# JingyunLiang/HCFlow

Measured on AMD Instinct MI355X. Metric: HR images/sec (inverse sample) DIV2K x4 160px LR, higher is better.
Workload: dtype f32 via f16x3 split (hi/lo f16 products, f32 accumulate); 1 GPU; SR_DF2K_4X inverse sampling (netG reverse=True), batch 16/GPU, LR 160x160 -> HR 640x640, tau=0.8, eps on device, output all-gather over RCCL for N>1; global_batch=16, lr_size=160, parallelism=dp1, streams_per_gpu=2

## Files before the change

hcflow_amd/csrc/hcf_conv_wino.h:

```cpp
#pragma once
#include <hip/hip_runtime.h>
#include <stdint.h>
#include <string.h>
#include <math.h>
#include <type_traits>
#include <vector>

namespace hcf {
namespace wino {

constexpr int TW = 32, TH = 8, HWP = TW + 2, HHP = TH + 2;
constexpr int A_REAL_PIECES = HHP * HWP * 4;
constexpr int A_BYTES = 22 * 1024;
constexpr int W_BYTES = 16 * 2 * 2 * 32 * 16;
constexpr int STAGE = A_BYTES + W_BYTES;
constexpr int X_BYTES = 10240;
constexpr int S0_OFF = 0, X_OFF = STAGE, S1_OFF = STAGE + X_BYTES, TAB_OFF = S1_OFF + STAGE;
constexpr int LDS_BYTES = TAB_OFF + 512;
constexpr float UNSPLIT = 1.f / 2048.f;

struct Src { const float* p; int cs, c0, n; };
struct Args {
  Src src[3];
  int nsrc;
// ... 128 lines not shown
  const int R = px >> 2, sl = (px & 3) * 4 + part;
  return R * 256 + ((sl ^ ((R & 7) << 1)) << 4);
}


namespace v2 {
constexpr int TH2 = 16, HH2 = TH2 + 2;
constexpr int A2_REAL = HH2 * HWP * 4;
constexpr int A2_BYTES = 39 * 1024;
constexpr int STAGE2 = A2_BYTES + W_BYTES;
constexpr int TAB2_OFF = 2 * STAGE2;
constexpr int LDS2_BYTES = TAB2_OFF + 512;
constexpr int FB2_OFF = LDS2_BYTES;
constexpr int LDS2S_BYTES = FB2_OFF + 512 * 16 + 64;
constexpr int ROWB = HWP * 64;
__host__ __device__ constexpr int a2_off(int row, int x, int part) {
  return row * ROWB + (x >> 2) * 256 + (((((x & 3) * 4 + part)) ^ ((x >> 2) & 7)) << 4);
}
}

typedef _Float16 f16x2 __attribute__((ext_vector_type(2)));
typedef uint32_t u32x4 __attribute__((ext_vector_type(4)));
__device__ __forceinline__ void split8(const float (&v)[8], u32x4& h, u32x4& l) {
#pragma unroll
  for (int i = 0; i < 4; ++i) {
    const f16x2 hh = {(_Float16)v[2 * i], (_Float16)v[2 * i + 1]};
    h[i] = __builtin_bit_cast(uint32_t, hh);
    uint32_t lo;
    asm("v_fma_mixlo_f16 %0, %1, -1.0, %2 op_sel_hi:[1,0,0]" : "=v"(lo) : "v"(h[i]), "v"(v[2 * i]));
    asm("v_fma_mixhi_f16 %0, %1, -1.0, %2 op_sel:[1,0,0] op_sel_hi:[1,0,0]" : "+v"(lo) : "v"(h[i]), "v"(v[2 * i + 1]));
// ... 28 lines not shown
}

typedef uint32_t u32x2 __attribute__((ext_vector_type(2)));
__device__ __forceinline__ void split4(const f32x4& v, u32x2& h, u32x2& l) {
#pragma unroll
  for (int i = 0; i < 2; ++i) {
    const f16x2 hh = {(_Float16)v[2 * i], (_Float16)v[2 * i + 1]};
    h[i] = __builtin_bit_cast(uint32_t, hh);
    uint32_t lo;
    asm("v_fma_mixlo_f16 %0, %1, -1.0, %2 op_sel_hi:[1,0,0]" : "=v"(lo) : "v"(h[i]), "v"(v[2 * i]));
    asm("v_fma_mixhi_f16 %0, %1, -1.0, %2 op_sel:[1,0,0] op_sel_hi:[1,0,0]" : "+v"(lo) : "v"(h[i]), "v"(v[2 * i + 1]));
    l[i] = lo;
  }
}

template <int RES, bool SC = false>
__global__ __launch_bounds__(512, 1) void conv_wino2_kernel(const Args a, const int nunits) {
  using namespace v2;
  extern __shared__ __attribute__((aligned(16))) char lds[];
  const int tid = threadIdx.x, lane = tid & 63, half = lane >> 5, li = lane & 31;
  const int wave = __builtin_amdgcn_readfirstlane(tid >> 6);
  const int xp = wave & 1, tg = wave >> 1;
  const int H = a.H, W = a.W, ntn = a.ntile_n, nchunk = a.nchunk;
  const int tiles_x = (W + TW - 1) / TW, tiles_y = (H + TH2 - 1) / TH2;

  const bool w7 = (wave == 7);
  const int padpix = a.B * H * W;
  int upix[5];
#pragma unroll
  for (int j = 0; j < 5; ++j) upix[j] = padpix;
  uint32_t partpk = 0;
#pragma unroll
  for (int j = 0; j < 5; ++j) {
// ... 52 lines not shown
  {                                                                                                \
    const int p16_ = (int)((pp_ >> (2 * (J))) & 0x30u);                                            \
    const int vo_ = (int)__umul24((unsigned)upix[J], (unsigned)csb_) + p16_;                       \
    W2_DMA(rsa_, vo_, so_, DST);                                                                   \
  }
#define W2_ISSUE(J0, J1, STG)                                                                      \
  {                                                                                                \
    char* const sb_ = lds + (STG) * STAGE2 + wave * 1024;                                          \
    _Pragma("unroll") for (int j_ = (J0); j_ < (J1); ++j_) {                                       \
      if (j_ < 4) W2_A_SLOT(j_ < 5 ? j_ : 0, sb_ + j_ * 8192)                                      \
      else if (j_ == 4) { if (!w7) W2_A_SLOT(4, sb_ + 4 * 8192) else W2_DMA(rsw, wvo, ws_, sb_ + 4 * 8192); } \
      else if (j_ < 8) W2_DMA(rsw, wvo, ws_ + (8 * j_ + wave - 39) * 1024, sb_ + j_ * 8192);       \
      else if (!w7) W2_DMA(rsw, wvo, ws_ + (8 * 8 + wave - 39) * 1024, sb_ + 8 * 8192);            \
    }                                                                                              \
  }

  const int trow = li >> 4, tcol = li & 15;
  int poff[4];
#pragma unroll
  for (int j = 0; j < 4; ++j) poff[j] = a2_off(4 * tg + 2 * trow, 2 * tcol + j, 2 * half);
  const int rowP = xp ? ROWB : 0, rowS = xp ? 3 * ROWB : 2 * ROWB;
  const float sg = __builtin_bit_cast(float, __builtin_amdgcn_readfirstlane(__builtin_bit_cast(int, xp ? -1.f : 1.f)));
  const int fw = A2_BYTES + half * 512 + li * 16 + xp * (8 * 4 * 512);

  float in_s = 1.f, out_s = 1.f;
  int in_max_bits = 0;
  if (SC) input_scales(a.in_max, in_s, out_s, in_max_bits);
  constexpr bool FBK = SC && RES == 0;
  const bool fb = FBK && a.fb_y != nullptr;
  if (tid < 64) {
    const float sc_ = (tid < 32 * ntn) ? a.scale[tid] : 1.f, bi_ = (tid < 32 * ntn) ? a.bias[tid] : 0.f;
    reinterpret_cast<float*>(lds + TAB2_OFF)[tid] = bi_ * sc_;
    reinterpret_cast<float*>(lds + TAB2_OFF)[64 + tid] = sc_ * UNSPLIT * out_s;
  }
  if (FBK) {
    if (fb) {
      *reinterpret_cast<f32x4*>(lds + FB2_OFF + tid * 16) = f32x4{0.f, 0.f, 0.f, 0.f};
      if (tid == 0) *reinterpret_cast<int*>(lds + FB2_OFF + 512 * 16) = 0;
    }
  }
  int u = blockIdx.x;
  if (u >= nunits) return;
#if defined(WINO_PROF)
  unsigned long long pw[8] = {0, 0, 0, 0, 0, 0, 0, 0};
  const unsigned long long pw_t0 = __builtin_readcyclecounter();
#endif
  W2_SETUP_UNIT(u)
  W2_CHUNK_SCALARS()
  W2_ISSUE(0, 9, 0)
  ++uc;
  int g = 0;
  const float slope = a.act == 1 ? 0.f : a.act == 2 ? 0.2f : 1.f;

  while (true) {
    f32x16 acc[8];
#pragma unroll
    for (int p = 0; p < 8; ++p)
#pragma unroll
      for (int r = 0; r < 16; ++r) acc[p][r] = 0.f;
    const int eb = ub, ey0 = uy0, ex0 = ux0, ent = unt;
    const int un = u + gridDim.x;

    for (int c = 0; c < nchunk; ++c, ++g) {
      const int stg = g & 1;
#if defined(WINO_PROF)
      const unsigned long long q0 = __builtin_readcyclecounter();
#endif
      asm volatile("s_waitcnt vmcnt(0)" ::: "memory");
#if defined(WINO_PROF)
      const unsigned long long q1 = __builtin_readcyclecounter();
#endif
      __builtin_amdgcn_s_barrier();
#if defined(WINO_PROF)
      const unsigned long long q2 = __builtin_readcyclecounter();
      pw[0] += q1 - q0; pw[1] += q2 - q1;
#endif
      if (c + 1 == nchunk) {
        if (un < nunits) W2_SETUP_UNIT(un)
        else {
          uc = 0; unt = 0;
#pragma unroll
          for (int j = 0; j < 5; ++j) upix[j] = padpix;
        }
      }
      W2_CHUNK_SCALARS()
      const char* const sb = lds + stg * STAGE2;
      const int so = stg ^ 1;
#define W2_LOAD_ROW(D, OFF)                                                                        \
  _Pragma("unroll") for (int j = 0; j < 4; ++j) {                                                  \
    const f32x4 x0_ = *reinterpret_cast<const f32x4*>(sb + poff[j] + (OFF));                       \
    const f32x4 x1_ = *reinterpret_cast<const f32x4*>(sb + (poff[j] ^ 16) + (OFF));                \
    _Pragma("unroll") for (int k = 0; k < 4; ++k) { D[j][k] = x0_[k]; D[j][4 + k] = x1_[k]; }      \
  }
#define W2_V(NU, T, K) (((NU) == 0) ? T[0][K] - T[2][K] : ((NU) == 1) ? T[1][K] + T[2][K] : ((NU) == 2) ? T[1][K] - T[2][K] : T[1][K] - T[3][K])
#define W2_MFMA(P, WW, VX) acc[P] = __builtin_amdgcn_mfma_f32_32x32x16_f16(WW, __builtin_bit_cast(f16x8, VX), acc[P], 0, 0, 0);
#define W2_XI(I, T)                                                                                \
  _Pragma("unroll") for (int nu = 0; nu < 4; ++nu) {                                               \
    float v_[8];                                                                                   \
    _Pragma("unroll") for (int k = 0; k < 8; ++k) v_[k] = W2_V(nu, T, k);                          \
    u32x4 vh_, vl_;                                                                                \
    if (SC) split8s(v_, in_s, vh_, vl_); else split8(v_, vh_, vl_);                                \
    const f16x8 w1_ = *reinterpret_cast<const f16x8*>(sb + fw + (((I) * 4 + nu) * 4) * 512);       \
    const f16x8 w2_ = *reinterpret_cast<const f16x8*>(sb + fw + (((I) * 4 + nu) * 4 + 2) * 512);   \
    W2_MFMA((I) * 4 + nu, w1_, vh_)                                                                \
    W2_MFMA((I) * 4 + nu, w2_, vh_)                                                                \
    W2_MFMA((I) * 4 + nu, w1_, vl_)                                                                \
  }
      float t_[4][8];
      {
        float ra[4][8], rc[4][8];
        W2_LOAD_ROW(ra, rowP)
        W2_LOAD_ROW(rc, 2 * ROWB)
        W2_ISSUE(0, 3, so)
#pragma unroll
        for (int j = 0; j < 4; ++j)
#pragma unroll
          for (int k = 0; k < 8; ++k) t_[j][k] = ra[j][k] - rc[j][k];
      }
      W2_XI(0, t_)
      W2_ISSUE(3, 6, so)
      {
        float ra[4][8], rc[4][8];
        W2_LOAD_ROW(ra, ROWB)
        W2_LOAD_ROW(rc, rowS)
#pragma unroll
        for (int j = 0; j < 4; ++j)
#pragma unroll
          for (int k = 0; k < 8; ++k) t_[j][k] = fmaf(sg, rc[j][k], ra[j][k]);
      }
      W2_ISSUE(6, 9, so)
      ++uc;
      W2_XI(1, t_)
#if defined(WINO_PROF)
      pw[6] += __builtin_readcyclecounter() - q2;
#endif
#undef W2_XI
#undef W2_MFMA
#undef W2_V
#undef W2_LOAD_ROW
    }

#if defined(WINO_PROF)
    const unsigned long long qe0 = __builtin_readcyclecounter();
#endif
    float chk = 0.f;
    f32x4 fbs = {0.f, 0.f, 0.f, 0.f};
    float fbm = 0.f;
    {
      char* const xbuf = lds + ((g - 1) & 1) * STAGE2 + tg * 16384;
      const int p8 = lane >> 3, qd = (lane >> 1) & 3, hd = lane & 1;
      const int wpos = (half * 32 + ((li + 4 * half) & 31)) * 16;
      const int wpos1 = (half * 32 + ((li + 4 * half + 8) & 31)) * 16;
      const int cb = ent * 32 + 8 * qd + 4 * hd;
      const f32x4 bs = *reinterpret_cast<const f32x4*>(lds + TAB2_OFF + cb * 4);
      const f32x4 ms = *reinterpret_cast<const f32x4*>(lds + TAB2_OFF + 256 + cb * 4);
      const bool second = (RES == 0) && a.out2 != nullptr && cb >= a.out2_split;
      const float slope_l = second ? (a.act2 == 1 ? 0.f : a.act2 == 2 ? 0.2f : 1.f) : slope;
      __builtin_amdgcn_s_barrier();
#pragma unroll
      for (int oa = 0; oa < 2; ++oa) {
        f32x4 rv1[2][2], rv2[2][2];
        size_t pixs[2][2];
        bool oks[2][2];
        int rpos[2];
#pragma unroll
        for (int sgrp = 0; sgrp < 2; ++sgrp) {
          const int patch = 16 * xp + 8 * sgrp + p8, prow = patch >> 4, pcol = patch & 15;
          rpos[sgrp] = (hd * 32 + ((patch + 4 * hd + 8 * (qd & 1)) & 31)) * 16 + qd * 1024;
#pragma unroll
          for (int ob = 0; ob < 2; ++ob) {
            const int yy = ey0 + 4 * tg + 2 * prow + oa, xx = ex0 + 2 * pcol + ob;
            oks[sgrp][ob] = yy < H && xx < W;
            pixs[sgrp][ob] = (size_t)((size_t)eb * H + (yy < H ? yy : H - 1)) * W + (xx < W ? xx : W - 1);
            if (RES == 1 || RES == 2) rv1[sgrp][ob] = *reinterpret_cast<const f32x4*>(a.res1 + pixs[sgrp][ob] * a.res1_cs + a.res1_c0 + cb);
            if (RES == 2) rv2[sgrp][ob] = *reinterpret_cast<const f32x4*>(a.res2 + pixs[sgrp][ob] * a.res2_cs + a.res2_c0 + cb);
            if (RES == 3) rv1[sgrp][ob] = *reinterpret_cast<const f32x4*>(a.pre + pixs[sgrp][ob] * a.pre_cs + a.pre_c0 + cb);
            if (FBK) { if (fb) rv1[sgrp][ob] = *reinterpret_cast<const f32x4*>(a.fb_y + pixs[sgrp][ob] * a.fb_y_cs + a.fb_y_c0 + cb); }
          }
        }
        if (oa == 1) __builtin_amdgcn_s_barrier();
#pragma unroll
        for (int q = 0; q < 4; ++q) {
          f32x4 P[2];
#pragma unroll
          for (int e = 0; e < 4; ++e) {
            const int r = 4 * q + e;
            float R[2][2];
#pragma unroll
            for (int i = 0; i < 2; ++i) {
              R[i][0] = acc[i * 4 + 0][r] + acc[i * 4 + 1][r] + acc[i * 4 + 2][r];
              R[i][1] = acc[i * 4 + 1][r] - acc[i * 4 + 2][r] - acc[i * 4 + 3][r];
            }
#pragma unroll
            for (int bb = 0; bb < 2; ++bb)
              P[bb][e] = (oa == 0) ? (xp ? R[0][bb] : R[0][bb] + R[1][bb]) : (xp ? -R[0][bb] - R[1][bb] : R[1][bb]);
          }
          char* const wbq = xbuf + ((xp * 2) * 4 + q) * 1024 + ((q & 1) ? wpos1 : wpos);
          *reinterpret_cast<f32x4*>(wbq) = P[0];
          *reinterpret_cast<f32x4*>(wbq + 4096) = P[1];
        }
        __builtin_amdgcn_s_barrier();
#pragma unroll
        for (int sgrp = 0; sgrp < 2; ++sgrp)
#pragma unroll
          for (int ob = 0; ob < 2; ++ob) {
            const f32x4 y0 = *reinterpret_cast<const f32x4*>(xbuf + ((0 * 2 + ob) * 4) * 1024 + rpos[sgrp]);
            const f32x4 y1 = *reinterpret_cast<const f32x4*>(xbuf + ((1 * 2 + ob) * 4) * 1024 + rpos[sgrp]);
            f32x4 v;
#pragma unroll
            for (int e = 0; e < 4; ++e) {
              const float yv = y0[e] + y1[e];
              chk = fmaf(yv, 0.f, chk);
              float z = fmaf(yv, ms[e], bs[e]);
              if (RES == 3) z = fmaf(rv1[sgrp][ob][e], ms[e] * 2048.f, z);
              v[e] = fmaxf(z, slope_l * z);
              if (RES == 1 || RES == 2) v[e] = fmaf(v[e], a.rs1, rv1[sgrp][ob][e]);
// ... 48 lines not shown
        }
      }
      if (tid == 0) {
        const int m = *reinterpret_cast<const int*>(lds + FB2_OFF + 512 * 16), m2 = max(m, in_max_bits);
        if (a.fb_max && m) atomicMax(reinterpret_cast<int*>(a.fb_max), m);
        if (a.fb_max2 && m2) atomicMax(reinterpret_cast<int*>(a.fb_max2), m2);
      }
    }
  }
#if defined(WINO_PROF)
  if (a.dbg && lane == 0 && (blockIdx.x & 31) == 17) {
    atomicAdd(a.dbg + 0, pw[0]); atomicAdd(a.dbg + 1, pw[1]); atomicAdd(a.dbg + 2, __builtin_readcyclecounter() - pw_t0);
    atomicAdd(a.dbg + 3, pw[3]); atomicAdd(a.dbg + 4, 1ull); atomicAdd(a.dbg + 5, pw[5]); atomicAdd(a.dbg + 6, pw[6]);
  }
#endif
#undef W2_SETUP_UNIT
#undef W2_DMA
#undef W2_A_SLOT
#undef W2_ISSUE
#undef W2_CHUNK_SCALARS
}

namespace v4 {
constexpr int TH4 = 8, HH4 = TH4 + 2;
constexpr int A4_BYTES = 22 * 1024;
constexpr int W4L_BYTES = 48 * 1024;
constexpr int W4_OFF0 = 2 * A4_BYTES;
constexpr int X4_SPARE = 19 * 1024;
constexpr int W4_OFF1 = W4_OFF0 + W4L_BYTES + X4_SPARE;
constexpr int TAB4_OFF = W4_OFF1 + W4L_BYTES;
constexpr int LDS4_BYTES = TAB4_OFF + 1024;
constexpr int NPIECE4 = 22 + 48;
}

// ... 346 lines not shown
    a.clk[3] = __builtin_amdgcn_s_memrealtime();
  }
  f16x8 w11[4];
  W4_SETUP_UNIT(u)
  W4_CHUNK_SCALARS()
  W4_ISSUE_A(0)
  W4_ISSUE_W(2, 9, 0)
#pragma unroll
  for (int nu = 0; nu < 4; ++nu) W4_LOAD_W11(nu)
  ++uc;
  int g = 0;
  const float slope = a.act == 1 ? 0.f : a.act == 2 ? 0.2f : 1.f;
  const float slope2 = a.act2 == 1 ? 0.f : a.act2 == 2 ? 0.2f : 1.f;
  const float slope_f = a.f_act == 1 ? 0.f : a.f_act == 2 ? 0.2f : 1.f;

  while (true) {
    f32x16 acc[4][2];
#pragma unroll
    for (int p = 0; p < 4; ++p)
#pragma unroll
      for (int n = 0; n < 2; ++n)
#pragma unroll
        for (int r = 0; r < 16; ++r) acc[p][n][r] = 0.f;
    const int eb = ub, ey0 = uy0, ex0 = ux0;
    const int un = u + gridDim.x;

    for (int c = 0; c < nchunk; ++c, ++g) {
      const int stg = g & 1;
#if defined(WINO_PROF)
      const unsigned long long q0 = __builtin_readcyclecounter();
#endif
      if (c > 0 || g == 0 || a.top_wait) asm volatile("s_waitcnt vmcnt(0)" ::: "memory");
#if defined(WINO_PROF)
      const unsigned long long q1 = __builtin_readcyclecounter();
#endif
      __builtin_amdgcn_s_barrier();
#if defined(WINO_PROF)
      const unsigned long long q2 = __builtin_readcyclecounter();
      pw[0] += q1 - q0; pw[1] += q2 - q1;
      if (c == 0 && g > 0) { pw[21] += q1 - q0; pw[22] += q2 - q1; pw[23] += 1; }
#endif
#pragma unroll
      for (int nu = 0; nu < 4; ++nu) asm volatile("" : "+v"(w11[nu]));
      if (c + 1 == nchunk) {
        if (un < nunits) W4_SETUP_UNIT(un)
        else {
          uc = 0;
#pragma unroll
          for (int j = 0; j < 3; ++j) upix[j] = padpix;
        }
      }
      W4_CHUNK_SCALARS()
      W4_ISSUE_A((g + 1) & 1)
      float t_[4][8];
      {
        const char* const ib = lds + (g & 1) * A4_BYTES;
        float ra[4][8], rb[4][8];
#pragma unroll
        for (int j = 0; j < 4; ++j) {
          const f32x4 x0_ = *reinterpret_cast<const f32x4*>(ib + poff[j] + offA);
          const f32x4 x1_ = *reinterpret_cast<const f32x4*>(ib + (poff[j] ^ 16) + offA);
          const f32x4 y0_ = *reinterpret_cast<const f32x4*>(ib + poff[j] + offB);
          const f32x4 y1_ = *reinterpret_cast<const f32x4*>(ib + (poff[j] ^ 16) + offB);
#pragma unroll
          for (int k = 0; k < 4; ++k) { ra[j][k] = x0_[k]; ra[j][4 + k] = x1_[k]; rb[j][k] = y0_[k]; rb[j][4 + k] = y1_[k]; }
        }
#pragma unroll
        for (int j = 0; j < 4; ++j)
#pragma unroll
          for (int k = 0; k < 8; ++k) t_[j][k] = fmaf(sg, rb[j][k], ra[j][k]);
      }
#if defined(WINO_PROF)
      const unsigned long long q3 = __builtin_readcyclecounter();
      pw[5] += q3 - q2;
#endif
      const char* const wb = lds + (stg ? W4_OFF1 : W4_OFF0) + fw;
#define W4_V(NU, K) (((NU) == 0) ? t_[0][K] - t_[2][K] : ((NU) == 1) ? t_[1][K] + t_[2][K] : ((NU) == 2) ? t_[1][K] - t_[2][K] : t_[1][K] - t_[3][K])
#define W4_MFMA(P, N, WW, VX) acc[P][N] = __builtin_amdgcn_mfma_f32_32x32x16_f16(WW, __builtin_bit_cast(f16x8, VX), acc[P][N], 0, 0, 0);
#pragma unroll
      for (int nu = 0; nu < 4; ++nu) {
        float v_[8];
#pragma unroll
        for (int k = 0; k < 8; ++k) v_[k] = W4_V(nu, k);
        u32x4 vh_, vl_;
        if (SC) split8s(v_, in_s, vh_, vl_); else split8(v_, vh_, vl_);
        const f16x8 w00 = *reinterpret_cast<const f16x8*>(wb + (nu * 3 + 0) * 1024);
        const f16x8 w01 = *reinterpret_cast<const f16x8*>(wb + (nu * 3 + 1) * 1024);
        const f16x8 w10 = *reinterpret_cast<const f16x8*>(wb + (nu * 3 + 2) * 1024);
        W4_MFMA(nu, 0, w00, vh_)
        W4_MFMA(nu, 1, w10, vh_)
        W4_MFMA(nu, 0, w01, vh_)
        W4_MFMA(nu, 1, w11[nu], vh_)
        W4_MFMA(nu, 0, w00, vl_)
        W4_MFMA(nu, 1, w10, vl_)
        if (nu == 0) { W4_ISSUE_W(2, 5, stg ^ 1) }
        else if (nu == 1) { W4_ISSUE_W(5, 7, stg ^ 1) }
        else if (nu == 2) { W4_ISSUE_W(7, 9, stg ^ 1) }
        W4_LOAD_W11(nu)
      }
      ++uc;
#if defined(WINO_PROF)
      pw[6] += __builtin_readcyclecounter() - q3;
#endif
#undef W4_V
#undef W4_MFMA
    }

#if defined(WINO_PROF)
    const unsigned long long qe0 = __builtin_readcyclecounter();
#endif
    int lane_e = lane;
    asm volatile("" : "+v"(lane_e));
    wino64_epilogue<RES>(a, lds, TAB4_OFF, lds + (((g - 1) & 1) ? W4_OFF0 + W4L_BYTES : W4_OFF0), acc, eb, ey0, ex0, H, W, slope, slope2, slope_f, wave, lane_e
#if defined(WINO_PROF)
                         , pw
#endif
                         );
#if defined(WINO_PROF)
    pw[3] += __builtin_readcyclecounter() - qe0;
#endif
    u = un;
    if (u >= nunits) break;
  }
  if (a.clk != nullptr && blockIdx.x == 0 && tid == 0) {
    a.clk[0] += __builtin_readcyclecounter() - a.clk[2];
    a.clk[1] += __builtin_amdgcn_s_memrealtime() - a.clk[3];
  }
#if defined(WINO_PROF)
  if (a.dbg && lane == 0 && (blockIdx.x & 31) == 17) {
    atomicAdd(a.dbg + 0, pw[0]); atomicAdd(a.dbg + 1, pw[1]); atomicAdd(a.dbg + 2, __builtin_readcyclecounter() - pw_t0);
    atomicAdd(a.dbg + 3, pw[3]); atomicAdd(a.dbg + 4, 1ull); atomicAdd(a.dbg + 5, pw[5]); atomicAdd(a.dbg + 6, pw[6]);
    atomicAdd(a.dbg + 7, pw[7]);
    for (int i = 8; i < 24; ++i) atomicAdd(a.dbg + i, pw[i]);
  }
#endif
#undef W4_SETUP_UNIT
#undef W4_DMA
#undef W4_A_SLOT
#undef W4_ISSUE_A
#undef W4_ISSUE_W
#undef W4_LOAD_W11
#undef W4_CHUNK_SCALARS
}


static inline int launch(const Args& a, int ncu, hipStream_t st, int version = 2) {
  if (a.nsrc < 1 || a.nsrc > 3 || !a.wpack || !a.bias || !a.scale || !a.ovf || !a.zeros || !a.out || a.nchunk < 1) return -1;
  if (a.ntile_n < 1 || a.ntile_n > 2 || (a.cout & 3)) return -6;
  int kt = 0;
  for (int i = 0; i < a.nsrc; ++i) {
// ... 6 lines not shown
  if (a.res1 && (((a.res1_cs | a.res1_c0) & 3) || (reinterpret_cast<uintptr_t>(a.res1) & 15))) return -6;
  if (a.res2 && (((a.res2_cs | a.res2_c0) & 3) || (reinterpret_cast<uintptr_t>(a.res2) & 15))) return -6;
  if (a.res2 && !a.res1) return -1;
  if ((long long)a.B * a.H * a.W >= (1LL << 24)) return -6;
  if (version == 4 && (a.ntile_n != 2 || a.cout > 64)) return -6;
  if (version == 4) {
    const int cs_[4] = {a.out_cs, a.out2 ? a.out2_cs : 0, a.res1 ? a.res1_cs : 0, a.res2 ? a.res2_cs : 0};
    for (int i = 0; i < 4; ++i)
      if (cs_[i] < 0 || (long long)(a.W + 1) * cs_[i] >= 0x7fffffffLL) return -6;
  }
  const int th = (version == 2) ? v2::TH2 : (version == 4) ? v4::TH4 : TH;
  const int tiles_x = (a.W + TW - 1) / TW, tiles_y = (a.H + th - 1) / th;
  const long long nunits = (long long)a.B * tiles_x * tiles_y * (version == 4 ? 1 : a.ntile_n);
  if (nunits < 1 || nunits > 0x7fffffffLL) return -1;
  const unsigned grid = (unsigned)(nunits < ncu ? nunits : ncu);
  static bool attr_dev[64][3][8] = {};
  int dev_ = 0;
  if (hipGetDevice(&dev_) != hipSuccess || dev_ < 0 || dev_ >= 64) return -2;
  bool (&attr)[3][8] = attr_dev[dev_];
  if (a.pre && (version != 2 || a.res1 || a.res2 || ((a.pre_cs | a.pre_c0) & 3) || (reinterpret_cast<uintptr_t>(a.pre) & 15))) return -6;
  if (a.out2 && (a.res1 || a.pre || ((a.out2_cs | a.out2_c0) & 3) || (reinterpret_cast<uintptr_t>(a.out2) & 15))) return -6;
  if (a.out2 && version != 4 && (version != 2 || a.ntile_n != 1 || a.out2_split != 16)) return -6;
  if (a.f_w && (version != 4 || a.res1 || a.res2 || a.out2 || !a.f_bias || !a.f_scale || (reinterpret_cast<uintptr_t>(a.f_w) & 15))) return -6;
  const int res = (a.pre || a.f_w) ? 3 : a.res2 ? 2 : a.res1 ? 1 : 0;
  const bool sc = a.in_max != nullptr;
  if (sc && (res > 1 || a.out2 || (version != 2 && version != 4))) return -6;
  if (a.fb_y && (!sc || version != 2 || res != 0 || a.ntile_n != 1 || !a.fb_part || ((a.fb_y_cs | a.fb_y_c0) & 3) ||
                 (reinterpret_cast<uintptr_t>(a.fb_y) & 15))) return -6;
  const int ldsb = (version == 2) ? (sc ? v2::LDS2S_BYTES : v2::LDS2_BYTES) : (version == 4) ? v4::LDS4_BYTES : LDS_BYTES;
  const int vi = (version == 2) ? 1 : (version == 4) ? 2 : 0;
  const int ai = res + (sc ? 4 : 0);
  auto go = [&](auto fn, int threads) {
    if (!attr[vi][ai]) {
      if (hipFuncSetAttribute(reinterpret_cast<const void*>(fn), hipFuncAttributeMaxDynamicSharedMemorySize, ldsb) != hipSuccess) return -2;
      attr[vi][ai] = true;
    }
    hipLaunchKernelGGL(fn, dim3(grid), dim3(threads), ldsb, st, a, (int)nunits);
    return hipGetLastError() == hipSuccess ? 0 : -2;
  };
  if (sc && version == 4) return res == 0 ? go(conv_wino4_kernel<0, true>, 512) : go(conv_wino4_kernel<1, true>, 512);
  if (sc && version == 2) return res == 0 ? go(conv_wino2_kernel<0, true>, 512) : go(conv_wino2_kernel<1, true>, 512);
  if (version == 4) {
    if (res == 0) return go(conv_wino4_kernel<0>, 512);
    if (res == 1) return go(conv_wino4_kernel<1>, 512);
    if (res == 3) return go(conv_wino4_kernel<3>, 512);
    return go(conv_wino4_kernel<2>, 512);
  }
  if (version == 2) {
    if (res == 0) return go(conv_wino2_kernel<0>, 512);
    if (res == 1) return go(conv_wino2_kernel<1>, 512);
    if (res == 3) return go(conv_wino2_kernel<3>, 512);
    return go(conv_wino2_kernel<2>, 512);
  }
  return -6;
}
#endif

}
}
```

hcflow_amd/csrc/hcf_conv_wino.hip:

```cpp
#include "hcf_common.h"
#include <cstdlib>
#include "hcf_conv_wino.h"
#include "hcf_pack_index.h"
#include <atomic>

namespace hcf {

size_t pack_conv_weights_wino(const float* w, int cin, int cout, const int* srcs, int nsrc, std::vector<float>& out, int min_cin_arg) {
  out.clear();
  static const int min_cin_env = getenv("HCF_WINO_MIN_CIN") ? atoi(getenv("HCF_WINO_MIN_CIN")) : 64;
  const int min_cin = min_cin_arg >= 0 ? min_cin_arg : min_cin_env;
  if (!w || cin < min_cin || (cout != 32 && cout != 64) || nsrc < 1 || nsrc > 3) return 0;
  int sum = 0;
  for (int i = 0; i < nsrc; ++i) {
    if (srcs[i] < 16 || (srcs[i] & 15)) return 0;
    sum += srcs[i];
  }
  if (sum != cin) return 0;
  std::vector<uint16_t> pk;
  if (!(cout == 64 ? wino::pack_weights_wino64(w, cin, cout, pk) : wino::pack_weights_wino(w, cin, cout, pk))) return 0;
  out.resize((pk.size() * 2 + 3) / 4);
  memcpy(out.data(), pk.data(), pk.size() * 2);
  return pk.size() * 2;
}

// ... 185 lines not shown
```

hcflow_amd/csrc/hcf_engine_run.inc:

```

  hipStream_t st = nullptr;
  bool dry() const { return arena.dry; }

  struct Buf {
    float* p; int C; int cs;
    View v(int c0, int n, int up = 0) const { return mkview(p, cs, c0, n, up); }
    View all() const { return mkview(p, cs, 0, C, 0); }
  };
  Buf alloc(int B, int H, int W, int C) {
    Buf b;
    b.C = C;
    b.cs = ru4(C);
    b.p = arena.alloc((size_t)B * H * W * b.cs);
    return b;
  }

  int B_ = 0;

  bool can_fuse_fcn(const Conv& c1, const Conv& c2, const View* z1 = nullptr) const {
    static const bool off = getenv("HCF_NO_FUSE_FCN") != nullptr;
    if (off) return false;
    if (taping) return false;
    if (z1 && ((z1->cs | z1->c0) & 3) != 0) return false;
    return use_f16 && c1.wpack16 && c2.wpack16 && c1.taps == 9 && c2.taps == 1 && c1.cout == 64 && c2.cout == 64 &&
// ... 320 lines not shown
    a.mat = nullptr;
    if (partial && s.mode == CPL_AFFINE) {
      a.partial = partial + pslot;
      a.partial_stride = pstride;
      pslot += step_blocks_per_sample(H, W);
    }
    HCF_LAUNCH(launch_step_couple_fwd(a, st));
  }

  bool tape_fat = false;
  void run_rdb(const Rdb& r, View xin, const Buf& grow, int H, int W, View out, View res2, float rs2, const Buf* fatp = nullptr) {
    const int gc = cfg.rrdb_gc;
    const bool fat_ok = fatp && fatp->p && use_f16 && (!taping || tape_fat) && !(g_f16x3_ablation & 256) &&
                        (gc == 16 || conv_wino_rounds_ok(B_, H, W, 2)) && conv_wino_rounds_ok(B_, H, W, 1) &&
                        wino_offsets_ok(H, W, std::max(std::max(xin.cs, grow.cs), fatp->cs));
    static const long long fat12_pixels = getenv("HCF_FAT12_PIXELS") ? atoll(getenv("HCF_FAT12_PIXELS")) : 40000;
    const bool use_fat[2] = {fat_ok && r.fat[0] && (gc == 16 || (long long)H * W <= fat12_pixels), fat_ok && r.fat[1]};
    ConvOpt last;
    last.res1 = xin; last.rs1 = 0.2f; last.res2 = res2; last.rs2 = rs2;
    if (use_fat[0] || use_fat[1]) {
      for (int j = 0; j < 2; ++j) {
        std::vector<View> srcs;
        srcs.push_back(xin);
        if (j > 0) srcs.push_back(grow.v(0, 2 * j * gc));
        if (use_fat[j]) {
          const FatExtra fa = {fatp->v(0, gc), ACT_NONE, false};
          ConvOpt oa; oa.fat = &fa;
          run_conv(r.ca[j], srcs, H, W, grow.v(2 * j * gc, gc), oa);
          const FatExtra fb = {View(), ACT_NONE, true};
          ConvOpt ob; ob.res1 = fatp->v(0, gc); ob.fat = &fb;
          run_conv(r.cb[j], {grow.v(2 * j * gc, gc)}, H, W, grow.v((2 * j + 1) * gc, gc), ob);
        } else {
// ... 338 lines not shown
```

Measured before the change: 135.9 HR images/s.

## Add lean two-chunk Winograd conv variant with reshaped LDS staging and early loads

```diff
diff --git a/hcflow_amd/csrc/hcf_conv_wino.h b/hcflow_amd/csrc/hcf_conv_wino.h
--- a/hcflow_amd/csrc/hcf_conv_wino.h
+++ b/hcflow_amd/csrc/hcf_conv_wino.h
@@ -166,6 +166,13 @@
 constexpr int FB2_OFF = LDS2_BYTES;
 constexpr int LDS2S_BYTES = FB2_OFF + 512 * 16 + 64;
 constexpr int ROWB = HWP * 64;
+constexpr int XL_OFF = STAGE2;
+constexpr int XL_SPARE = 17920;
+constexpr int S1L_OFF = XL_OFF + XL_SPARE;
+constexpr int XL_W1_PIECES = (XL_OFF + 65536 - (S1L_OFF + A2_BYTES) + 1023) / 1024;
+constexpr int TABL_OFF = S1L_OFF + STAGE2;
+constexpr int LDS2L_BYTES = TABL_OFF + 512;
+static_assert(XL_W1_PIECES <= 9 && (S1L_OFF & 255) == 0 && LDS2L_BYTES <= 160 * 1024, "lean layout");
 __host__ __device__ constexpr int a2_off(int row, int x, int part) {
   return row * ROWB + (x >> 2) * 256 + (((((x & 3) * 4 + part)) ^ ((x >> 2) & 7)) << 4);
 }
@@ -224,9 +231,11 @@
   }
 }
 
-template <int RES, bool SC = false>
+template <int RES, bool SC = false, bool LEAN = false>
 __global__ __launch_bounds__(512, 1) void conv_wino2_kernel(const Args a, const int nunits) {
   using namespace v2;
+  static_assert(!(LEAN && SC), "the lean form has no room for the fused epilogue backward's sums");
+  constexpr int TAB = LEAN ? TABL_OFF : TAB2_OFF;
   extern __shared__ __attribute__((aligned(16))) char lds[];
   const int tid = threadIdx.x, lane = tid & 63, half = lane >> 5, li = lane & 31;
   const int wave = __builtin_amdgcn_readfirstlane(tid >> 6);
@@ -309,6 +318,22 @@
       else if (!w7) W2_DMA(rsw, wvo, ws_ + (8 * 8 + wave - 39) * 1024, sb_ + 8 * 8192);            \
     }                                                                                              \
   }
+#define W2_ISSUE_L(J0, J1, STG, FULL)                                                              \
+  {                                                                                                \
+    char* const sb_ = lds + ((STG) ? S1L_OFF : 0) + wave * 1024;                                   \
+    _Pragma("unroll") for (int j_ = (J0); j_ < (J1); ++j_) {                                       \
+      if (j_ < 4) W2_A_SLOT(j_ < 5 ? j_ : 0, sb_ + j_ * 8192)                                      \
+      else if (j_ == 4) { if (!w7) W2_A_SLOT(4, sb_ + 4 * 8192) else if ((STG) || (FULL)) W2_DMA(rsw, wvo, ws_, sb_ + 4 * 8192); } \
+      else if (j_ == 5) { if ((STG) || (FULL)) W2_DMA(rsw, wvo, ws_ + (8 * j_ + wave - 39) * 1024, sb_ + j_ * 8192); } \
+      else if (j_ < 8) { if (FULL) W2_DMA(rsw, wvo, ws_ + (8 * j_ + wave - 39) * 1024, sb_ + j_ * 8192); } \
+      else if (!w7) { if (FULL) W2_DMA(rsw, wvo, ws_ + (8 * 8 + wave - 39) * 1024, sb_ + 8 * 8192); } \
+    }                                                                                              \
+  }
+#define W2_ISSUE_C(J0, J1, FIRST)                                                                  \
+  {                                                                                                \
+    if (LEAN) { if (FIRST) W2_ISSUE_L(J0, J1, 1, g == 0) else W2_ISSUE_L(J0, J1, 0, false) }       \
+    else W2_ISSUE(J0, J1, so)                                                                      \
+  }
 
   const int trow = li >> 4, tcol = li & 15;
   int poff[4];
@@ -325,8 +350,8 @@
   const bool fb = FBK && a.fb_y != nullptr;
   if (tid < 64) {
     const float sc_ = (tid < 32 * ntn) ? a.scale[tid] : 1.f, bi_ = (tid < 32 * ntn) ? a.bias[tid] : 0.f;
-    reinterpret_cast<float*>(lds + TAB2_OFF)[tid] = bi_ * sc_;
-    reinterpret_cast<float*>(lds + TAB2_OFF)[64 + tid] = sc_ * UNSPLIT * out_s;
+    reinterpret_cast<float*>(lds + TAB)[tid] = bi_ * sc_;
+    reinterpret_cast<float*>(lds + TAB)[64 + tid] = sc_ * UNSPLIT * out_s;
   }
   if (FBK) {
     if (fb) {
@@ -342,45 +367,16 @@
 #endif
   W2_SETUP_UNIT(u)
   W2_CHUNK_SCALARS()
-  W2_ISSUE(0, 9, 0)
+  if (LEAN) W2_ISSUE_L(0, 9, 0, true) else W2_ISSUE(0, 9, 0)
   ++uc;
   int g = 0;
   const float slope = a.act == 1 ? 0.f : a.act == 2 ? 0.2f : 1.f;
 
-  while (true) {
-    f32x16 acc[8];
-#pragma unroll
-    for (int p = 0; p < 8; ++p)
-#pragma unroll
-      for (int r = 0; r < 16; ++r) acc[p][r] = 0.f;
-    const int eb = ub, ey0 = uy0, ex0 = ux0, ent = unt;
-    const int un = u + gridDim.x;
-
-    for (int c = 0; c < nchunk; ++c, ++g) {
-      const int stg = g & 1;
 #if defined(WINO_PROF)
-      const unsigned long long q0 = __builtin_readcyclecounter();
-#endif
-      asm volatile("s_waitcnt vmcnt(0)" ::: "memory");
-#if defined(WINO_PROF)
-      const unsigned long long q1 = __builtin_readcyclecounter();
-#endif
-      __builtin_amdgcn_s_barrier();
-#if defined(WINO_PROF)
-      const unsigned long long q2 = __builtin_readcyclecounter();
-      pw[0] += q1 - q0; pw[1] += q2 - q1;
-#endif
-      if (c + 1 == nchunk) {
-        if (un < nunits) W2_SETUP_UNIT(un)
-        else {
-          uc = 0; unt = 0;
-#pragma unroll
-          for (int j = 0; j < 5; ++j) upix[j] = padpix;
-        }
-      }
-      W2_CHUNK_SCALARS()
-      const char* const sb = lds + stg * STAGE2;
-      const int so = stg ^ 1;
+#define W2_PROF(...) __VA_ARGS__
+#else
+#define W2_PROF(...)
+#endif
 #define W2_LOAD_ROW(D, OFF)                                                                        \
   _Pragma("unroll") for (int j = 0; j < 4; ++j) {                                                  \
     const f32x4 x0_ = *reinterpret_cast<const f32x4*>(sb + poff[j] + (OFF));                       \
@@ -389,7 +385,8 @@
   }
 #define W2_V(NU, T, K) (((NU) == 0) ? T[0][K] - T[2][K] : ((NU) == 1) ? T[1][K] + T[2][K] : ((NU) == 2) ? T[1][K] - T[2][K] : T[1][K] - T[3][K])
 #define W2_MFMA(P, WW, VX) acc[P] = __builtin_amdgcn_mfma_f32_32x32x16_f16(WW, __builtin_bit_cast(f16x8, VX), acc[P], 0, 0, 0);
-#define W2_XI(I, T)                                                                                \
+#define W2_MFMA0(P, WW, VX) acc[P] = __builtin_amdgcn_mfma_f32_32x32x16_f16(WW, __builtin_bit_cast(f16x8, VX), zero16, 0, 0, 0);
+#define W2_XI(I, T, FIRST)                                                                         \
   _Pragma("unroll") for (int nu = 0; nu < 4; ++nu) {                                               \
     float v_[8];                                                                                   \
     _Pragma("unroll") for (int k = 0; k < 8; ++k) v_[k] = W2_V(nu, T, k);                          \
@@ -397,43 +394,67 @@
     if (SC) split8s(v_, in_s, vh_, vl_); else split8(v_, vh_, vl_);                                \
     const f16x8 w1_ = *reinterpret_cast<const f16x8*>(sb + fw + (((I) * 4 + nu) * 4) * 512);       \
     const f16x8 w2_ = *reinterpret_cast<const f16x8*>(sb + fw + (((I) * 4 + nu) * 4 + 2) * 512);   \
-    W2_MFMA((I) * 4 + nu, w1_, vh_)                                                                \
+    if (FIRST) { W2_MFMA0((I) * 4 + nu, w1_, vh_) } else { W2_MFMA((I) * 4 + nu, w1_, vh_) }       \
     W2_MFMA((I) * 4 + nu, w2_, vh_)                                                                \
     W2_MFMA((I) * 4 + nu, w1_, vl_)                                                                \
   }
-      float t_[4][8];
-      {
-        float ra[4][8], rc[4][8];
-        W2_LOAD_ROW(ra, rowP)
-        W2_LOAD_ROW(rc, 2 * ROWB)
-        W2_ISSUE(0, 3, so)
-#pragma unroll
-        for (int j = 0; j < 4; ++j)
-#pragma unroll
-          for (int k = 0; k < 8; ++k) t_[j][k] = ra[j][k] - rc[j][k];
-      }
-      W2_XI(0, t_)
-      W2_ISSUE(3, 6, so)
-      {
-        float ra[4][8], rc[4][8];
-        W2_LOAD_ROW(ra, ROWB)
-        W2_LOAD_ROW(rc, rowS)
-#pragma unroll
-        for (int j = 0; j < 4; ++j)
-#pragma unroll
-          for (int k = 0; k < 8; ++k) t_[j][k] = fmaf(sg, rc[j][k], ra[j][k]);
-      }
-      W2_ISSUE(6, 9, so)
-      ++uc;
-      W2_XI(1, t_)
-#if defined(WINO_PROF)
-      pw[6] += __builtin_readcyclecounter() - q2;
-#endif
-#undef W2_XI
-#undef W2_MFMA
-#undef W2_V
-#undef W2_LOAD_ROW
-    }
+#define W2_CHUNK(FIRST)                                                                            \
+  {                                                                                                \
+    const int stg = LEAN ? ((FIRST) ? 0 : 1) : (g & 1);                                            \
+    W2_PROF(const unsigned long long q0 = __builtin_readcyclecounter();)                           \
+     \
+     \
+    if (!LEAN || !(FIRST) || g == 0 || a.top_wait) asm volatile("s_waitcnt vmcnt(0)" ::: "memory"); \
+    W2_PROF(const unsigned long long q1 = __builtin_readcyclecounter();)                           \
+    __builtin_amdgcn_s_barrier();                                                                  \
+    W2_PROF(const unsigned long long q2 = __builtin_readcyclecounter(); pw[0] += q1 - q0; pw[1] += q2 - q1;) \
+    if (LEAN ? !(FIRST) : (c + 1 == nchunk)) {                                                     \
+      if (un < nunits) W2_SETUP_UNIT(un)                                                           \
+      else {                                                                                       \
+        uc = 0; unt = 0;                                                                           \
+        _Pragma("unroll") for (int j = 0; j < 5; ++j) upix[j] = padpix;                            \
+      }                                                                                            \
+    }                                                                                              \
+    W2_CHUNK_SCALARS()                                                                             \
+    const char* const sb = lds + (LEAN ? (stg ? S1L_OFF : 0) : stg * STAGE2);                      \
+    const int so = stg ^ 1;                                                                        \
+    (void)so;                                                                                      \
+    float t_[4][8];                                                                                \
+    {                                                                                              \
+      float ra[4][8], rc[4][8];                                                                    \
+      W2_LOAD_ROW(ra, rowP)                                                                        \
+      W2_LOAD_ROW(rc, 2 * ROWB)                                                                    \
+      W2_ISSUE_C(0, 3, FIRST)                                                                      \
+      _Pragma("unroll") for (int j = 0; j < 4; ++j)                                                \
+        _Pragma("unroll") for (int k = 0; k < 8; ++k) t_[j][k] = ra[j][k] - rc[j][k];              \
+    }                                                                                              \
+    W2_XI(0, t_, FIRST)                                                                            \
+    W2_ISSUE_C(3, 6, FIRST)                                                                        \
+    {                                                                                              \
+      float ra[4][8], rc[4][8];                                                                    \
+      W2_LOAD_ROW(ra, ROWB)                                                                        \
+      W2_LOAD_ROW(rc, rowS)                                                                        \
+      _Pragma("unroll") for (int j = 0; j < 4; ++j)                                                \
+        _Pragma("unroll") for (int k = 0; k < 8; ++k) t_[j][k] = fmaf(sg, rc[j][k], ra[j][k]);     \
+    }                                                                                              \
+    W2_ISSUE_C(6, 9, FIRST)                                                                        \
+    ++uc;                                                                                          \
+    W2_XI(1, t_, FIRST)                                                                            \
+    W2_PROF(pw[6] += __builtin_readcyclecounter() - q2;)                                           \
+  }
+  const f32x16 zero16 = {0.f, 0.f, 0.f, 0.f, 0.f, 0.f, 0.f, 0.f, 0.f, 0.f, 0.f, 0.f, 0.f, 0.f, 0.f, 0.f};
+
+  while (true) {
+    f32x16 acc[8];
+    const int eb = ub, ey0 = uy0, ex0 = ux0, ent = unt;
+    const int un = u + gridDim.x;
+
+    int c = 0;
+    W2_CHUNK(1)
+    ++g;
+    if (LEAN) { W2_CHUNK(0) ++g; }
+    else for (c = 1; c < nchunk; ++c, ++g) W2_CHUNK(0)
+    (void)c;
 
 #if defined(WINO_PROF)
     const unsigned long long qe0 = __builtin_readcyclecounter();
@@ -442,15 +463,29 @@
     f32x4 fbs = {0.f, 0.f, 0.f, 0.f};
     float fbm = 0.f;
     {
-      char* const xbuf = lds + ((g - 1) & 1) * STAGE2 + tg * 16384;
+      char* const xbuf = lds + (LEAN ? XL_OFF : ((g - 1) & 1) * STAGE2) + tg * 16384;
       const int p8 = lane >> 3, qd = (lane >> 1) & 3, hd = lane & 1;
       const int wpos = (half * 32 + ((li + 4 * half) & 31)) * 16;
       const int wpos1 = (half * 32 + ((li + 4 * half + 8) & 31)) * 16;
       const int cb = ent * 32 + 8 * qd + 4 * hd;
-      const f32x4 bs = *reinterpret_cast<const f32x4*>(lds + TAB2_OFF + cb * 4);
-      const f32x4 ms = *reinterpret_cast<const f32x4*>(lds + TAB2_OFF + 256 + cb * 4);
+      const f32x4 bs = *reinterpret_cast<const f32x4*>(lds + TAB + cb * 4);
+      const f32x4 ms = *reinterpret_cast<const f32x4*>(lds + TAB + 256 + cb * 4);
       const bool second = (RES == 0) && a.out2 != nullptr && cb >= a.out2_split;
       const float slope_l = second ? (a.act2 == 1 ? 0.f : a.act2 == 2 ? 0.2f : 1.f) : slope;
+      f32x4 pv[2][2][2];
+      if (LEAN && RES == 3) {
+#pragma unroll
+        for (int oa = 0; oa < 2; ++oa)
+#pragma unroll
+          for (int sgrp = 0; sgrp < 2; ++sgrp)
+#pragma unroll
+            for (int ob = 0; ob < 2; ++ob) {
+              const int patch = 16 * xp + 8 * sgrp + p8, prow = patch >> 4, pcol = patch & 15;
+              const int yy = ey0 + 4 * tg + 2 * prow + oa, xx = ex0 + 2 * pcol + ob;
+              const size_t pix = (size_t)((size_t)eb * H + (yy < H ? yy : H - 1)) * W + (xx < W ? xx : W - 1);
+              pv[oa][sgrp][ob] = *reinterpret_cast<const f32x4*>(a.pre + pix * a.pre_cs + a.pre_c0 + cb);
+            }
+      }
       __builtin_amdgcn_s_barrier();
 #pragma unroll
       for (int oa = 0; oa < 2; ++oa) {
@@ -469,7 +504,10 @@
             pixs[sgrp][ob] = (size_t)((size_t)eb * H + (yy < H ? yy : H - 1)) * W + (xx < W ? xx : W - 1);
             if (RES == 1 || RES == 2) rv1[sgrp][ob] = *reinterpret_cast<const f32x4*>(a.res1 + pixs[sgrp][ob] * a.res1_cs + a.res1_c0 + cb);
             if (RES == 2) rv2[sgrp][ob] = *reinterpret_cast<const f32x4*>(a.res2 + pixs[sgrp][ob] * a.res2_cs + a.res2_c0 + cb);
-            if (RES == 3) rv1[sgrp][ob] = *reinterpret_cast<const f32x4*>(a.pre + pixs[sgrp][ob] * a.pre_cs + a.pre_c0 + cb);
+            if (RES == 3) {
+              if (LEAN) rv1[sgrp][ob] = pv[oa][sgrp][ob];
+              else rv1[sgrp][ob] = *reinterpret_cast<const f32x4*>(a.pre + pixs[sgrp][ob] * a.pre_cs + a.pre_c0 + cb);
+            }
             if (FBK) { if (fb) rv1[sgrp][ob] = *reinterpret_cast<const f32x4*>(a.fb_y + pixs[sgrp][ob] * a.fb_y_cs + a.fb_y_c0 + cb); }
           }
         }
@@ -495,6 +533,15 @@
           *reinterpret_cast<f32x4*>(wbq + 4096) = P[1];
         }
         __builtin_amdgcn_s_barrier();
+        if (LEAN && oa == 0) {
+          asm volatile("s_waitcnt vmcnt(0)" ::: "memory");
+          if (RES == 3) {
+#pragma unroll
+            for (int i = 0; i < 8; ++i) asm volatile("" : "+v"(pv[i >> 2][(i >> 1) & 1][i & 1]));
+#pragma unroll
+            for (int i = 0; i < 4; ++i) asm volatile("" : "+v"(rv1[i >> 1][i & 1]));
+          }
+        }
 #pragma unroll
         for (int sgrp = 0; sgrp < 2; ++sgrp)
 #pragma unroll
@@ -573,10 +620,19 @@
     atomicAdd(a.dbg + 3, pw[3]); atomicAdd(a.dbg + 4, 1ull); atomicAdd(a.dbg + 5, pw[5]); atomicAdd(a.dbg + 6, pw[6]);
   }
 #endif
+#undef W2_CHUNK
+#undef W2_XI
+#undef W2_MFMA0
+#undef W2_MFMA
+#undef W2_V
+#undef W2_LOAD_ROW
+#undef W2_PROF
 #undef W2_SETUP_UNIT
 #undef W2_DMA
 #undef W2_A_SLOT
 #undef W2_ISSUE
+#undef W2_ISSUE_L
+#undef W2_ISSUE_C
 #undef W2_CHUNK_SCALARS
 }
 
@@ -953,97 +1009,82 @@
   const float slope2 = a.act2 == 1 ? 0.f : a.act2 == 2 ? 0.2f : 1.f;
   const float slope_f = a.f_act == 1 ? 0.f : a.f_act == 2 ? 0.2f : 1.f;
 
+#if defined(WINO_PROF)
+#define W4_PROF(...) __VA_ARGS__
+#else
+#define W4_PROF(...)
+#endif
+#define W4_V(NU, K) (((NU) == 0) ? t_[0][K] - t_[2][K] : ((NU) == 1) ? t_[1][K] + t_[2][K] : ((NU) == 2) ? t_[1][K] - t_[2][K] : t_[1][K] - t_[3][K])
+#define W4_MFMA(P, N, WW, VX) acc[P][N] = __builtin_amdgcn_mfma_f32_32x32x16_f16(WW, __builtin_bit_cast(f16x8, VX), acc[P][N], 0, 0, 0);
+#define W4_MFMA0(P, N, WW, VX) acc[P][N] = __builtin_amdgcn_mfma_f32_32x32x16_f16(WW, __builtin_bit_cast(f16x8, VX), zero16, 0, 0, 0);
+#define W4_CHUNK(FIRST)                                                                            \
+  {                                                                                                \
+    const int stg = g & 1;                                                                         \
+    W4_PROF(const unsigned long long q0 = __builtin_readcyclecounter();)                           \
+    if (!(FIRST) || g == 0 || a.top_wait) asm volatile("s_waitcnt vmcnt(0)" ::: "memory");         \
+    W4_PROF(const unsigned long long q1 = __builtin_readcyclecounter();)                           \
+    __builtin_amdgcn_s_barrier();                                                                  \
+    W4_PROF(const unsigned long long q2 = __builtin_readcyclecounter(); pw[0] += q1 - q0; pw[1] += q2 - q1;             \
+            if ((FIRST) && g > 0) { pw[21] += q1 - q0; pw[22] += q2 - q1; pw[23] += 1; })          \
+    _Pragma("unroll") for (int nu = 0; nu < 4; ++nu) asm volatile("" : "+v"(w11[nu]));    \
+    if (c + 1 == nchunk) {                                                                         \
+      if (un < nunits) W4_SETUP_UNIT(un)                                                           \
+      else {                                                                                       \
+        uc = 0;                                                                                    \
+        _Pragma("unroll") for (int j = 0; j < 3; ++j) upix[j] = padpix;                            \
+      }                                                                                            \
+    }                                                                                              \
+    W4_CHUNK_SCALARS()                                                                             \
+    W4_ISSUE_A((g + 1) & 1)                        \
+    float t_[4][8];                                                                                \
+    {                                                                                              \
+      const char* const ib = lds + (g & 1) * A4_BYTES;                                             \
+      float ra[4][8], rb[4][8];                                                                    \
+      _Pragma("unroll") for (int j = 0; j < 4; ++j) {                                              \
+        const f32x4 x0_ = *reinterpret_cast<const f32x4*>(ib + poff[j] + offA);                    \
+        const f32x4 x1_ = *reinterpret_cast<const f32x4*>(ib + (poff[j] ^ 16) + offA);             \
+        const f32x4 y0_ = *reinterpret_cast<const f32x4*>(ib + poff[j] + offB);                    \
+        const f32x4 y1_ = *reinterpret_cast<const f32x4*>(ib + (poff[j] ^ 16) + offB);             \
+        _Pragma("unroll") for (int k = 0; k < 4; ++k) { ra[j][k] = x0_[k]; ra[j][4 + k] = x1_[k]; rb[j][k] = y0_[k]; rb[j][4 + k] = y1_[k]; } \
+      }                                                                                            \
+      _Pragma("unroll") for (int j = 0; j < 4; ++j)                                                \
+        _Pragma("unroll") for (int k = 0; k < 8; ++k) t_[j][k] = fmaf(sg, rb[j][k], ra[j][k]);     \
+    }                                                                                              \
+    W4_PROF(const unsigned long long q3 = __builtin_readcyclecounter(); pw[5] += q3 - q2;)         \
+    const char* const wb = lds + (stg ? W4_OFF1 : W4_OFF0) + fw;                                   \
+    _Pragma("unroll") for (int nu = 0; nu < 4; ++nu) {                                             \
+      float v_[8];                                                                                 \
+      _Pragma("unroll") for (int k = 0; k < 8; ++k) v_[k] = W4_V(nu, k);                           \
+      u32x4 vh_, vl_;                                                                              \
+      if (SC) split8s(v_, in_s, vh_, vl_); else split8(v_, vh_, vl_);                              \
+      const f16x8 w00 = *reinterpret_cast<const f16x8*>(wb + (nu * 3 + 0) * 1024);                 \
+      const f16x8 w01 = *reinterpret_cast<const f16x8*>(wb + (nu * 3 + 1) * 1024);                 \
+      const f16x8 w10 = *reinterpret_cast<const f16x8*>(wb + (nu * 3 + 2) * 1024);                 \
+      if (FIRST) { W4_MFMA0(nu, 0, w00, vh_) W4_MFMA0(nu, 1, w10, vh_) }                           \
+      else { W4_MFMA(nu, 0, w00, vh_) W4_MFMA(nu, 1, w10, vh_) }                                   \
+      W4_MFMA(nu, 0, w01, vh_)                                                                     \
+      W4_MFMA(nu, 1, w11[nu], vh_)                                                                 \
+      W4_MFMA(nu, 0, w00, vl_)                                                                     \
+      W4_MFMA(nu, 1, w10, vl_)                                                                     \
+      if (nu == 0) { W4_ISSUE_W(2, 5, stg ^ 1) }                                                   \
+      else if (nu == 1) { W4_ISSUE_W(5, 7, stg ^ 1) }                                              \
+      else if (nu == 2) { W4_ISSUE_W(7, 9, stg ^ 1) }                                              \
+      W4_LOAD_W11(nu)         \
+    }                                                                                              \
+    ++uc;                                                                                          \
+    W4_PROF(pw[6] += __builtin_readcyclecounter() - q3;)                                           \
+  }
+  const f32x16 zero16 = {0.f, 0.f, 0.f, 0.f, 0.f, 0.f, 0.f, 0.f, 0.f, 0.f, 0.f, 0.f, 0.f, 0.f, 0.f, 0.f};
+
   while (true) {
     f32x16 acc[4][2];
-#pragma unroll
-    for (int p = 0; p < 4; ++p)
-#pragma unroll
-      for (int n = 0; n < 2; ++n)
-#pragma unroll
-        for (int r = 0; r < 16; ++r) acc[p][n][r] = 0.f;
     const int eb = ub, ey0 = uy0, ex0 = ux0;
     const int un = u + gridDim.x;
 
-    for (int c = 0; c < nchunk; ++c, ++g) {
-      const int stg = g & 1;
-#if defined(WINO_PROF)
-      const unsigned long long q0 = __builtin_readcyclecounter();
-#endif
-      if (c > 0 || g == 0 || a.top_wait) asm volatile("s_waitcnt vmcnt(0)" ::: "memory");
-#if defined(WINO_PROF)
-      const unsigned long long q1 = __builtin_readcyclecounter();
-#endif
-      __builtin_amdgcn_s_barrier();
-#if defined(WINO_PROF)
-      const unsigned long long q2 = __builtin_readcyclecounter();
-      pw[0] += q1 - q0; pw[1] += q2 - q1;
-      if (c == 0 && g > 0) { pw[21] += q1 - q0; pw[22] += q2 - q1; pw[23] += 1; }
-#endif
-#pragma unroll
-      for (int nu = 0; nu < 4; ++nu) asm volatile("" : "+v"(w11[nu]));
-      if (c + 1 == nchunk) {
-        if (un < nunits) W4_SETUP_UNIT(un)
-        else {
-          uc = 0;
-#pragma unroll
-          for (int j = 0; j < 3; ++j) upix[j] = padpix;
-        }
-      }
-      W4_CHUNK_SCALARS()
-      W4_ISSUE_A((g + 1) & 1)
-      float t_[4][8];
-      {
-        const char* const ib = lds + (g & 1) * A4_BYTES;
-        float ra[4][8], rb[4][8];
-#pragma unroll
-        for (int j = 0; j < 4; ++j) {
-          const f32x4 x0_ = *reinterpret_cast<const f32x4*>(ib + poff[j] + offA);
-          const f32x4 x1_ = *reinterpret_cast<const f32x4*>(ib + (poff[j] ^ 16) + offA);
-          const f32x4 y0_ = *reinterpret_cast<const f32x4*>(ib + poff[j] + offB);
-          const f32x4 y1_ = *reinterpret_cast<const f32x4*>(ib + (poff[j] ^ 16) + offB);
-#pragma unroll
-          for (int k = 0; k < 4; ++k) { ra[j][k] = x0_[k]; ra[j][4 + k] = x1_[k]; rb[j][k] = y0_[k]; rb[j][4 + k] = y1_[k]; }
-        }
-#pragma unroll
-        for (int j = 0; j < 4; ++j)
-#pragma unroll
-          for (int k = 0; k < 8; ++k) t_[j][k] = fmaf(sg, rb[j][k], ra[j][k]);
-      }
-#if defined(WINO_PROF)
-      const unsigned long long q3 = __builtin_readcyclecounter();
-      pw[5] += q3 - q2;
-#endif
-      const char* const wb = lds + (stg ? W4_OFF1 : W4_OFF0) + fw;
-#define W4_V(NU, K) (((NU) == 0) ? t_[0][K] - t_[2][K] : ((NU) == 1) ? t_[1][K] + t_[2][K] : ((NU) == 2) ? t_[1][K] - t_[2][K] : t_[1][K] - t_[3][K])
-#define W4_MFMA(P, N, WW, VX) acc[P][N] = __builtin_amdgcn_mfma_f32_32x32x16_f16(WW, __builtin_bit_cast(f16x8, VX), acc[P][N], 0, 0, 0);
-#pragma unroll
-      for (int nu = 0; nu < 4; ++nu) {
-        float v_[8];
-#pragma unroll
-        for (int k = 0; k < 8; ++k) v_[k] = W4_V(nu, k);
-        u32x4 vh_, vl_;
-        if (SC) split8s(v_, in_s, vh_, vl_); else split8(v_, vh_, vl_);
-        const f16x8 w00 = *reinterpret_cast<const f16x8*>(wb + (nu * 3 + 0) * 1024);
-        const f16x8 w01 = *reinterpret_cast<const f16x8*>(wb + (nu * 3 + 1) * 1024);
-        const f16x8 w10 = *reinterpret_cast<const f16x8*>(wb + (nu * 3 + 2) * 1024);
-        W4_MFMA(nu, 0, w00, vh_)
-        W4_MFMA(nu, 1, w10, vh_)
-        W4_MFMA(nu, 0, w01, vh_)
-        W4_MFMA(nu, 1, w11[nu], vh_)
-        W4_MFMA(nu, 0, w00, vl_)
-        W4_MFMA(nu, 1, w10, vl_)
-        if (nu == 0) { W4_ISSUE_W(2, 5, stg ^ 1) }
-        else if (nu == 1) { W4_ISSUE_W(5, 7, stg ^ 1) }
-        else if (nu == 2) { W4_ISSUE_W(7, 9, stg ^ 1) }
-        W4_LOAD_W11(nu)
-      }
-      ++uc;
-#if defined(WINO_PROF)
-      pw[6] += __builtin_readcyclecounter() - q3;
-#endif
-#undef W4_V
-#undef W4_MFMA
-    }
+    int c = 0;
+    W4_CHUNK(1)
+    ++g;
+    for (c = 1; c < nchunk; ++c, ++g) W4_CHUNK(0)
 
 #if defined(WINO_PROF)
     const unsigned long long qe0 = __builtin_readcyclecounter();
@@ -1073,6 +1114,11 @@
     for (int i = 8; i < 24; ++i) atomicAdd(a.dbg + i, pw[i]);
   }
 #endif
+#undef W4_CHUNK
+#undef W4_MFMA0
+#undef W4_MFMA
+#undef W4_V
+#undef W4_PROF
 #undef W4_SETUP_UNIT
 #undef W4_DMA
 #undef W4_A_SLOT
@@ -1109,10 +1155,10 @@
   const long long nunits = (long long)a.B * tiles_x * tiles_y * (version == 4 ? 1 : a.ntile_n);
   if (nunits < 1 || nunits > 0x7fffffffLL) return -1;
   const unsigned grid = (unsigned)(nunits < ncu ? nunits : ncu);
-  static bool attr_dev[64][3][8] = {};
+  static bool attr_dev[64][4][8] = {};
   int dev_ = 0;
   if (hipGetDevice(&dev_) != hipSuccess || dev_ < 0 || dev_ >= 64) return -2;
-  bool (&attr)[3][8] = attr_dev[dev_];
+  bool (&attr)[4][8] = attr_dev[dev_];
   if (a.pre && (version != 2 || a.res1 || a.res2 || ((a.pre_cs | a.pre_c0) & 3) || (reinterpret_cast<uintptr_t>(a.pre) & 15))) return -6;
   if (a.out2 && (a.res1 || a.pre || ((a.out2_cs | a.out2_c0) & 3) || (reinterpret_cast<uintptr_t>(a.out2) & 15))) return -6;
   if (a.out2 && version != 4 && (version != 2 || a.ntile_n != 1 || a.out2_split != 16)) return -6;
@@ -1122,8 +1168,9 @@
   if (sc && (res > 1 || a.out2 || (version != 2 && version != 4))) return -6;
   if (a.fb_y && (!sc || version != 2 || res != 0 || a.ntile_n != 1 || !a.fb_part || ((a.fb_y_cs | a.fb_y_c0) & 3) ||
                  (reinterpret_cast<uintptr_t>(a.fb_y) & 15))) return -6;
-  const int ldsb = (version == 2) ? (sc ? v2::LDS2S_BYTES : v2::LDS2_BYTES) : (version == 4) ? v4::LDS4_BYTES : LDS_BYTES;
-  const int vi = (version == 2) ? 1 : (version == 4) ? 2 : 0;
+  const bool lean = version == 2 && !sc && a.nchunk == 2 && a.ntile_n == 1;
+  const int ldsb = lean ? v2::LDS2L_BYTES : (version == 2) ? (sc ? v2::LDS2S_BYTES : v2::LDS2_BYTES) : (version == 4) ? v4::LDS4_BYTES : LDS_BYTES;
+  const int vi = lean ? 3 : (version == 2) ? 1 : (version == 4) ? 2 : 0;
   const int ai = res + (sc ? 4 : 0);
   auto go = [&](auto fn, int threads) {
     if (!attr[vi][ai]) {
@@ -1141,6 +1188,12 @@
     if (res == 3) return go(conv_wino4_kernel<3>, 512);
     return go(conv_wino4_kernel<2>, 512);
   }
+  if (lean) {
+    if (res == 0) return go(conv_wino2_kernel<0, false, true>, 512);
+    if (res == 1) return go(conv_wino2_kernel<1, false, true>, 512);
+    if (res == 3) return go(conv_wino2_kernel<3, false, true>, 512);
+    return go(conv_wino2_kernel<2, false, true>, 512);
+  }
   if (version == 2) {
     if (res == 0) return go(conv_wino2_kernel<0>, 512);
     if (res == 1) return go(conv_wino2_kernel<1>, 512);
diff --git a/hcflow_amd/csrc/hcf_conv_wino.hip b/hcflow_amd/csrc/hcf_conv_wino.hip
--- a/hcflow_amd/csrc/hcf_conv_wino.hip
+++ b/hcflow_amd/csrc/hcf_conv_wino.hip
@@ -8,7 +8,8 @@
 
 size_t pack_conv_weights_wino(const float* w, int cin, int cout, const int* srcs, int nsrc, std::vector<float>& out, int min_cin_arg) {
   out.clear();
-  static const int min_cin_env = getenv("HCF_WINO_MIN_CIN") ? atoi(getenv("HCF_WINO_MIN_CIN")) : 64;
+  const char* const min_cin_s = getenv("HCF_WINO_MIN_CIN");
+  const int min_cin_env = min_cin_s ? atoi(min_cin_s) : 64;
   const int min_cin = min_cin_arg >= 0 ? min_cin_arg : min_cin_env;
   if (!w || cin < min_cin || (cout != 32 && cout != 64) || nsrc < 1 || nsrc > 3) return 0;
   int sum = 0;
diff --git a/hcflow_amd/csrc/hcf_engine_run.inc b/hcflow_amd/csrc/hcf_engine_run.inc
--- a/hcflow_amd/csrc/hcf_engine_run.inc
+++ b/hcflow_amd/csrc/hcf_engine_run.inc
@@ -358,8 +358,9 @@
     const bool fat_ok = fatp && fatp->p && use_f16 && (!taping || tape_fat) && !(g_f16x3_ablation & 256) &&
                         (gc == 16 || conv_wino_rounds_ok(B_, H, W, 2)) && conv_wino_rounds_ok(B_, H, W, 1) &&
                         wino_offsets_ok(H, W, std::max(std::max(xin.cs, grow.cs), fatp->cs));
-    static const long long fat12_pixels = getenv("HCF_FAT12_PIXELS") ? atoll(getenv("HCF_FAT12_PIXELS")) : 40000;
-    const bool use_fat[2] = {fat_ok && r.fat[0] && (gc == 16 || (long long)H * W <= fat12_pixels), fat_ok && r.fat[1]};
+    const char* const fat12_env = getenv("HCF_FAT12_PIXELS");
+    const long long fat12_pixels = fat12_env ? atoll(fat12_env) : -1;
+    const bool use_fat[2] = {fat_ok && r.fat[0] && (gc == 16 || fat12_pixels < 0 || (long long)H * W <= fat12_pixels), fat_ok && r.fat[1]};
     ConvOpt last;
     last.res1 = xin; last.rs1 = 0.2f; last.res2 = res2; last.rs2 = rs2;
     if (use_fat[0] || use_fat[1]) {
```

After: 137.2 HR images/s (median of 6 runs). About the same (+0.9%).
